# lxvm/AutoBZCore.jl

Hardware: AMD Instinct MI355X
Metric: k-point evals/sec (H(k)+eig) (higher is better)
Workload: dtype f64

## Files before the change

autobzcore.jl_amd/csrc/abz_internal.h:

```cpp
#pragma once
#include <hip/hip_ext.h>
#include <hip/hip_runtime.h>

#include <atomic>
#include <cstdint>
#include <cstdio>
#include <memory>
#include <string>
#include <vector>

#include "../../include/abzhip.h"
#include "dev_buf.h"
#include "ltm_block.h"
#include "plane_view.h"

namespace abz {
struct ProfScope;
struct RulePlan;

void set_error(const char* fmt, ...);
int catch_status() noexcept;

#define ABZ_CATCH_ALL \
    catch (...) { return abz::catch_status(); }
// ... 28 lines not shown
    SW_IPANEL_FMAC,
    SW_GGR_FUSED,
    SW_GGR_FUSE2,
    SW_GGR_UNIFORM,
    SW_IAI_SPECULATE,
    SW_IAI_PACKED,
    SW_IAI_POOL_MB,
    SW_IAI_DEVICE_INNER,
    SW_IAI_PANELS,
    SW_IAI_STATS,
    SW_HOST_THREADS,
    SW_AUTO_SWEEP_MAPPED,
    SW_LANE_KERNELS,
    SW_BIG_MFMA,
    SW_BIG_CHUNK_MB,
    SW_BIG_TRI_WAVES,
    SW_EIG_FOLD,
    SW_EIG_SPLIT,
    SW_IAI_LANES,
    SW_IAI_LANE_MIN,
    SW_CHAIN_FUSED,
    SW_EVAL_FUSED,
    SW_EVAL_PAIRS,
    SW_COUNT
};
int abz_switch(Switch s);

int stage_h2d(abz_ctx* ctx, void* dst_dev, const void* src_host, size_t bytes);
int stage_d2h(abz_ctx* ctx, void* dst_host, const void* src_dev, size_t bytes);
int mbox_reserve(abz_ctx* ctx);

int sweep_to_device(abz_ctx* ctx, const double* host, int n, const double** dev);

struct SumOut {
    double* host = nullptr;
    double* dev = nullptr;
    double2* map_dev = nullptr;
    const double2* map_host = nullptr;
};
int sum_target(abz_ctx* ctx, const SumOut& so, int64_t col0, int64_t ncols, double2** where);
int sum_deliver(abz_ctx* ctx, const SumOut& so, const double2* from, int64_t col0, int64_t ncols);

struct EnergyList {
    std::vector<int> perm;
    std::vector<double> Es, res;
    const double* dev = nullptr;
// ... 65 lines not shown
        so.map_dev = mbox_results<double2>(ctx, true);
        so.map_host = mbox_results<const double2>(ctx, false);
    }
    return so;
}
struct SeriesRule {
    int npt = 0, want = 0;
    std::vector<int32_t> syms;
    abz_rule* r = nullptr;
    uint64_t generation = 0;
    uint64_t stamp = 0;
};
}

struct abz_series {
    std::atomic<int> refs{1};
    bool closed = false;
    abz_ctx* ctx = nullptr;
    int d = 0, n = 0;
    int dims[ABZ_MAX_DIM] = {1, 1, 1};
    int first[ABZ_MAX_DIM] = {0, 0, 0};
    double period[ABZ_MAX_DIM] = {1, 1, 1};
    bool hermitian = false;
    int pivoting = ABZ_PIVOT_NONE;
    abz::DevBuf coef_pk;
    bool coef_pk_valid = false;
    abz::DevBuf coef;
    std::vector<abz_series*> lanes;
    abz::DevBuf pool[ABZ_MAX_DIM + 1];
    abz::DevBuf iai_pool[ABZ_MAX_DIM + 1];
    int64_t iai_used[ABZ_MAX_DIM + 1] = {0, 0, 0, 0};
    abz::DevBuf iai_io[6];
    abz_exchange_fn ex_fn = nullptr;
    void* ex_user = nullptr;
    int ex_rank = 0, ex_world = 1;
    void* iai_pin[5] = {nullptr, nullptr, nullptr, nullptr, nullptr};
    size_t iai_pin_cap[5] = {0, 0, 0, 0, 0};
    void* iai_pin_dev[5] = {nullptr, nullptr, nullptr, nullptr, nullptr};
    uint64_t generation = 0;
    std::vector<abz::SeriesRule> kept_rules;
    uint64_t kept_stamp = 0;
    std::vector<int> summed_once;
    uint64_t auto_hint_key = 0;
    int auto_hint_grids = 0;
    abz::DevBuf auto_io;
    void* auto_pin = nullptr;
// ... 104 lines not shown
                          int64_t L, int M3, int M2, int npt, int gbeg, int gcnt);

struct EvalSpec {
    int n;
    int M, first;
    double period;
    const double2* src;
    bool grid;
    int npt;
    int64_t nlines;
    const double2* tab;
    int64_t nk;
    const int64_t* run_start = nullptr;
    int64_t nruns = 0;
    const int64_t* parents;
    const int32_t* gi;
    const double* x;
    bool deriv;
    bool herm;
    bool packed = false;
    const double2* src2 = nullptr;
    const double2* phs2 = nullptr;
    int M2 = 0;
    PlaneView H;
    PlaneView E;
    PlaneView U;
};
int launch_eval(abz_ctx* ctx, const EvalSpec& es);
bool eval_packed_supported(int n, int M, int npt);
bool eval_fused_supported(int n, int64_t mnn, int M2, int npt, bool pairs = false);
int launch_pack_rows(abz_ctx* ctx, int n, int M, const double2* src, int64_t nrows, double2* out);
size_t packed_row_elems(int n, int M);
int series_ensure_packed(abz_series* s);

int launch_eig_planes(abz_ctx* ctx, int n, PlaneView H, PlaneView E, PlaneView U, int64_t nk);
int launch_velocity(abz_ctx* ctx, int n, PlaneView U, PlaneView dH, PlaneView Vj, int64_t nk);

struct ReduceSpec {
    int n, d, npt;
    int integrand;
    PlaneView H;
    PlaneView E;
    int64_t nk;
    const double* w;
    const int32_t* idx;
    int64_t k_offset = 0;
    bool herm = false;
    bool pivot = false;
    double params[4];
    const double* sweep_dev;
    int n_sweep;
    double scale;
// ... 238 lines not shown
```

autobzcore.jl_amd/csrc/api.cpp:

```cpp
#include <algorithm>
#include <atomic>
#include <cstdarg>
#include <chrono>
#include <cmath>
#include <cstring>
#include <map>
#include <mutex>
#include <numeric>
#include <thread>

#include "abz_internal.h"

namespace abz {

static thread_local std::string g_err;

void set_error(const char* fmt, ...) {
    char buf[1024];
    va_list ap;
    va_start(ap, fmt);
    vsnprintf(buf, sizeof(buf), fmt, ap);
    va_end(ap);
    g_err = buf;
}
// ... 40 lines not shown
    {"ABZ_IPANEL_FMAC", 1, "0: 16-lane panel kernel with separate pivot-row broadcasts"},
    {"ABZ_GGR_FUSED", 1, "0: GGR build by eigenvectors + one velocity launch per variable"},
    {"ABZ_GGR_FUSE2", 1, "0: fused GGR build reads level-1 families instead of contracting variable 2 itself"},
    {"ABZ_GGR_UNIFORM", 1, "0: GGR scans search the energy window even in equispaced lists"},
    {"ABZ_IAI_SPECULATE", 1, "0: nested IAI driver requests one panel per integral and round"},
    {"ABZ_IAI_PACKED", 1, "0: IAI chains on plain coefficient sets"},
    {"ABZ_IAI_POOL_MB", 0, "> 0: MB per chunk of level sets in the IAI driver (default: sized from free memory)"},
    {"ABZ_IAI_DEVICE_INNER", 1, "0: innermost GK loops driven from the host, one launch per round"},
    {"ABZ_IAI_PANELS", 1, "0: the level above the innermost one ships nodes instead of panels (GK rule of that level on the host)"},
    {"ABZ_IAI_STATS", 0, "1: per-solve statistics of the IAI driver on stderr"},
    {"ABZ_HOST_THREADS", 8, "host threads for the per-integral bookkeeping of IAI sweeps (capped at half the cores)"},
    {"ABZ_AUTO_SWEEP_MAPPED", 1, "0: abz_autoptr_solve* uploads its swept values instead of letting the kernels read the pinned host copy"},
    {"ABZ_LANE_KERNELS", 1, "0: 5...8-band rule builds / store-free sums on full grids through the 8-lane row kernels (test: same values)"},
    {"ABZ_BIG_MFMA", 0, "1: 33...64 bands: the level-1 evaluation of full grid lines as a real GEMM on v_mfma_f64_16x16x4_f64 (test: same values)"},
    {"ABZ_BIG_CHUNK_MB", 0, "33...64 bands: MB of scratch for the matrices of a chunk of nodes (0: 256, GGR builds 2048; tests set 1 to walk many chunks)"},
    {"ABZ_BIG_TRI_WAVES", 0, "33...64 bands: waves per node of the Householder tridiagonalisation (1, 2, 4: the same reflectors, another summation order; 0: two up to 44 bands, one up to 48, four above)"},
    {"ABZ_EIG_FOLD", 1, "0: 5...16-band rule builds evaluate the full level-1 series of a Hermitian model instead of the folded one"},
    {"ABZ_EIG_SPLIT", 1, "0: eigenvalues of 5...16-band rules by bisection inside the grid kernel instead of the per-lane QR kernel"},
    {"ABZ_IAI_LANES", 4, "lanes (host thread + stream each) a sweep of independent IAI solves is split over; 1: off"},
    {"ABZ_IAI_LANE_MIN", 16, "solves per lane below which a sweep is not split further"},
    {"ABZ_CHAIN_FUSED", 1, "0: 3-D full-grid chains contract variables 3 and 2 in two launches instead of contract_chain_kernel"},
    {"ABZ_EVAL_FUSED", 1, "0: 3-D full-grid rules (n <= 4) build level-1 sets with contract_chain_kernel instead of contracting variable 2 inside the grid kernel"},
    {"ABZ_EVAL_PAIRS", 1, "fused grid kernel, one grid line per half-wave: 1 where it takes fewer lane-rounds per line (Hermitian series), 0 never, 2 wherever supported (tests: same values)"},
};
}

int abz_switch(Switch s) {
    const char* e = getenv(g_switches[s].name);
    return (e && *e) ? atoi(e) : g_switches[s].dflt;
}

namespace {
struct Block {
    void* p;
    size_t cap;
    int device;
};
std::mutex g_pool_mutex;
std::vector<Block> g_pool;
size_t g_pool_bytes = 0;
std::atomic<int64_t> g_live_bytes{0};
std::atomic<int64_t> g_live_blocks{0};
size_t pool_limit() {
    static const size_t lim = (size_t)std::max(0, abz_switch(SW_POOL_MB)) << 20;
    return lim;
}
// ... 673 lines not shown
    return ABZ_OK;
} ABZ_CATCH_ALL

int abz_prof_reset(abz_ctx* ctx) try {
    ABZ_REQUIRE(ctx, "null ctx");
    int rc = prof_collect(ctx);
    for (auto& sl : ctx->prof_slots) {
        sl.ms = 0;
        sl.launches = 0;
    }
    return rc;
} ABZ_CATCH_ALL

int abz_prof_read(abz_ctx* ctx, int kernel_id, double* total_ms, int64_t* launches) try {
    ABZ_REQUIRE(ctx && kernel_id >= 0 && kernel_id < ABZ_K_COUNT, "bad profile slot");
    int rc = prof_collect(ctx);
    if (rc) return rc;
    if (total_ms) *total_ms = ctx->prof_slots[kernel_id].ms;
    if (launches) *launches = ctx->prof_slots[kernel_id].launches;
    return ABZ_OK;
} ABZ_CATCH_ALL

static bool detect_hermitian(const abz_series* s, const double* coef_reim);

int abz_series_create(abz_ctx* ctx, const double* coef_reim, int d, const int32_t* dims, const int32_t* first,
                      const double* period, int n, abz_series** out) try {
    ABZ_REQUIRE(ctx && coef_reim && dims && first && period && out, "abz_series_create: null argument");
    ABZ_REQUIRE(!ctx->closed, "abz_series_create: the context was destroyed");
    ABZ_REQUIRE(d >= 1 && d <= ABZ_MAX_DIM, "series dimension d = %d not in 1..%d", d, ABZ_MAX_DIM);
    ABZ_REQUIRE(n >= 1 && n <= ABZ_MAX_BANDS, "n = %d bands not in 1..%d", n, ABZ_MAX_BANDS);
    *out = nullptr;
    ABZ_HIP(hipSetDevice(ctx->device));
    std::unique_ptr<abz_series> s(new abz_series());
    s->ctx = ctx;
    s->d = d;
    s->n = n;
    for (int j = 0; j < d; ++j) {
        ABZ_REQUIRE(dims[j] >= 1 && period[j] > 0, "dims[%d] = %d / period = %g invalid", j, dims[j], period[j]);
        s->dims[j] = dims[j];
        s->first[j] = first[j];
        s->period[j] = period[j];
    }
    const size_t bytes = sizeof(double2) * (size_t)s->elems(d);
    if (s->coef.alloc(bytes)) return ABZ_ERR_NOMEM;
    hipError_t e = hipMemcpy(s->coef.p, coef_reim, bytes, hipMemcpyHostToDevice);
    if (e != hipSuccess) {
        set_error("coefficient upload failed: %s", hipGetErrorString(e));
        return ABZ_ERR_HIP;
    }
    s->hermitian = detect_hermitian(s.get(), coef_reim);
    ctx->refs += 1;
    *out = s.release();
    return ABZ_OK;
} ABZ_CATCH_ALL

static bool detect_hermitian(const abz_series* s, const double* coef_reim) {
    const int d = s->d, n = s->n;
    for (int j = 0; j < d; ++j)
        if (s->first[j] != -(s->dims[j] - 1) - s->first[j]) return false;
    int64_t nR = 1;
    for (int j = 0; j < d; ++j) nR *= s->dims[j];
    const int nn = n * n;
    for (int64_t r = 0; r < nR; ++r) {
        int64_t rem = r, mr = 0, mul = 1;
        for (int j = 0; j < d; ++j) {
            const int64_t i = rem % s->dims[j];
            rem /= s->dims[j];
            mr += (s->dims[j] - 1 - i) * mul;
            mul *= s->dims[j];
        }
        if (mr < r) continue;
        const double* A = coef_reim + 2 * r * nn;
        const double* B = coef_reim + 2 * mr * nn;
        for (int b = 0; b < n; ++b)
            for (int a = 0; a < n; ++a) {
                if (A[2 * (a + n * b)] != B[2 * (b + n * a)] || A[2 * (a + n * b) + 1] != -B[2 * (b + n * a) + 1])
                    return false;
            }
    }
    return true;
}

int abz_series_update(abz_series* s, const double* coef_reim) try {
    int rc = check_series(s);
    if (rc) return rc;
    ABZ_REQUIRE(coef_reim, "null coefficients");
    ABZ_HIP(hipSetDevice(s->ctx->device));
    ABZ_HIP(hipMemcpyAsync(s->coef.p, coef_reim, sizeof(double2) * (size_t)s->elems(s->d), hipMemcpyHostToDevice,
                           s->ctx->stream));
    ABZ_HIP(hipStreamSynchronize(s->ctx->stream));
    s->hermitian = detect_hermitian(s, coef_reim);
    s->coef_pk_valid = false;
    s->generation += 1;
    for (int64_t& u : s->iai_used) u = 0;
    for (abz_series* v : s->lanes) {
        v->hermitian = s->hermitian;
        v->coef_pk_valid = false;
        v->generation += 1;
    }
    return ABZ_OK;
} ABZ_CATCH_ALL

int abz_series_set_pivoting(abz_series* s, int mode) try {
    ABZ_REQUIRE(s, "abz_series_set_pivoting: null series");
    int rc = check_series(s);
    if (rc) return rc;
    ABZ_REQUIRE(mode == ABZ_PIVOT_NONE || mode == ABZ_PIVOT_PARTIAL, "abz_series_set_pivoting: mode %d is neither ABZ_PIVOT_NONE nor ABZ_PIVOT_PARTIAL", mode);
    s->pivoting = mode;
    for (abz_series* v : s->lanes) v->pivoting = mode;
    return ABZ_OK;
} ABZ_CATCH_ALL

int abz_series_get_pivoting(const abz_series* s, int* mode) try {
    ABZ_REQUIRE(s && mode, "abz_series_get_pivoting: null argument");
    ABZ_REQUIRE(!s->closed, "abz_series_get_pivoting: the series was destroyed");
    *mode = s->pivoting;
    return ABZ_OK;
} ABZ_CATCH_ALL

}

namespace abz {
int series_lane_views(abz_series* s, int count) {
    while ((int)s->lanes.size() < count) {
        abz_ctx* c = nullptr;
        int rc = abz_ctx_create(s->ctx->device, &c);
        if (rc) return rc;
        abz_series* v = new abz_series();
        v->ctx = c;
        v->d = s->d;
        v->n = s->n;
        for (int j = 0; j < ABZ_MAX_DIM; ++j) {
            v->dims[j] = s->dims[j];
            v->first[j] = s->first[j];
            v->period[j] = s->period[j];
        }
        v->hermitian = s->hermitian;
        v->pivoting = s->pivoting;
        v->coef = DevBuf::view_of(s->coef.p);
        c->refs += 1;
        s->lanes.push_back(v);
    }
    return ABZ_OK;
}
}

extern "C" {

static void series_drop_kept_rules(abz_series* s) {
    if (s->kept_rules.empty()) return;
    (void)hipSetDevice(s->ctx->device);
    (void)hipStreamSynchronize(s->ctx->stream);
    for (auto& k : s->kept_rules) delete k.r;
    s->kept_rules.clear();
    s->summed_once.clear();
}

int abz_series_destroy(abz_series* s) try {
    if (!s || s->closed) return ABZ_OK;
    series_drop_kept_rules(s);
// ... 173 lines not shown
        es.first = s->first[0];
        es.period = s->period[0];
        es.src = level1;
        if (level2) {
            es.src2 = level2;
            es.phs2 = rp->pd.phg[1].as<double2>();
            es.M2 = s->dims[1];
        }
        es.grid = r->full;
        es.npt = r->npt;
        es.nlines = r->full ? (d == 1 ? 1 : plan.nitems[1]) : 0;
        es.tab = tab;
        es.nk = r->nk;
        es.parents = r->full ? nullptr : rp->pd.parent[0].as<int64_t>();
        es.gi = r->full ? nullptr : rp->pd.gi[0].as<int32_t>();
        if (!r->full && plan.nruns > 0 && !plan.coords) {
            es.run_start = rp->pd.runs.as<int64_t>();
            es.nruns = plan.nruns;
        }
        es.x = nullptr;
        es.deriv = deriv;
        es.herm = s->hermitian;
        es.packed = packed_chain && !deriv && !Uout.base;
        es.H = Hout;
        es.E = Eout;
        es.U = Uout;
        return launch_eval(ctx, es);
    };
    const double2* level1 = nullptr;
    int rc;
    const int64_t line_elems = packed_chain ? (int64_t)packed_row_elems(n, s->dims[0]) : (int64_t)s->dims[0] * n * n;
    const bool ref_layout_large = s->hermitian && r->H.base && !r->H.compact && r->npt > 64;
    const bool eval_fused = r->full && d == 3 && n <= 4 && !(r->want & ABZ_WANT_VEL) && !Uv.base && rp->pd.phg[2].p && rp->pd.phg[1].p &&
                            !ref_layout_large &&
                            abz_switch(SW_CHAIN_FUSED) && abz_switch(SW_EVAL_FUSED) &&
                            contract_chain_fits(line_elems, s->dims[2], s->dims[1], r->npt, plan.outer_n) &&
                            eval_fused_supported(n, line_elems, s->dims[1], r->npt);
    if (eval_fused) {
        const double2* level2 = nullptr;
        if ((rc = build_chain(s, plan, rp->pd, tab, 0, &level2, 2, nullptr, packed_chain))) return rc;
        return run_eval(nullptr, false, r->H, r->E, PlaneView(), level2);
    }
    if ((rc = build_chain(s, plan, rp->pd, tab, 0, &level1, 1, nullptr, packed_chain))) return rc;
    if ((rc = run_eval(level1, false, r->H, vel_done ? PlaneView() : r->E, Uv))) return rc;
    if ((r->want & ABZ_WANT_VEL) && !vel_done) {
        for (int j = 1; j <= d; ++j) {
// ... 886 lines not shown
```

autobzcore.jl_amd/csrc/kernels.hip:

```cpp
#include "abz_internal.h"
#include "device_math.h"
#include "gk15.h"
#include "inner_adapt.h"
#include "packed_herm.h"

#include <cmath>
#include <cstring>
#include <type_traits>
#include <utility>
#include <cstdlib>

namespace abz {

static inline int64_t cdiv(int64_t a, int64_t b) { return (a + b - 1) / b; }

struct cplx_pod {
    double x, y;
};
typedef const cplx_pod __attribute__((address_space(4))) * cptr_t;
__device__ __forceinline__ cptr_t as_const(const double2* p) {
    return (cptr_t)(unsigned long long)p;
}

struct PhaseArgs {
// ... 442 lines not shown
        for (int a = 0; a < N; ++a) {
            H.re[a][b] = in[(int64_t)(2 * (a + N * b)) * v.pitch];
            H.im[a][b] = in[(int64_t)(2 * (a + N * b) + 1) * v.pitch];
        }
    }
}

struct EvalArgs {
    const double2* src;
    const double2* tab;
    const int64_t* parents;
    const int32_t* gi;
    const double* x;
    PlaneView H, E, U;
    int64_t nlines, nk;
    int64_t line0;
    int M, first, npt, deriv, herm;
    int nt;
    int pk;
    double inv_period;
    const double2* src2 = nullptr;
    const double2* phs2 = nullptr;
    int M2 = 0, bpk = 0;
};

template <bool NT>
__device__ __forceinline__ void store_f64(double* p, double v) {
    if constexpr (NT)
        __builtin_nontemporal_store(v, p);
    else
        *p = v;
}
template <int N, bool NT = false, bool HC = false>
__device__ __forceinline__ void store_planes_at(const CMat<N>& H, const PlaneView& v, int64_t line, int i1) {
    double* __restrict__ row = v.base + line * v.tile;
    const unsigned u = (unsigned)i1;
    if constexpr (HC) {
#pragma unroll
        for (int b = 0; b < N; ++b) {
#pragma unroll
            for (int a = 0; a <= b; ++a) {
                store_f64<NT>((row + (int64_t)(b * b + 2 * a) * v.pitch) + u, H.re[a][b]);
                if (a < b) store_f64<NT>((row + (int64_t)(b * b + 2 * a + 1) * v.pitch) + u, H.im[a][b]);
            }
        }
    } else {
#pragma unroll
        for (int b = 0; b < N; ++b) {
#pragma unroll
            for (int a = 0; a < N; ++a) {
                store_f64<NT>((row + (int64_t)(2 * (a + N * b)) * v.pitch) + u, H.re[a][b]);
                store_f64<NT>((row + (int64_t)(2 * (a + N * b) + 1) * v.pitch) + u, H.im[a][b]);
            }
        }
    }
}

template <int N, bool VEC = true>
__device__ __forceinline__ void eval_epilogue(const EvalArgs& a, CMat<N>& H, int64_t line, int i1) {
    if (a.H.base) {
        if (a.H.compact)
            store_planes_at<N, false, true>(H, a.H, line, i1);
        else
            store_planes_at<N>(H, a.H, line, i1);
    }
    if (a.E.base || (VEC && a.U.base)) {
        double e[N];
        CMat<N> V;
        if (VEC && a.U.base) {
            herm_eig<N, true>(H, e, V);
            store_planes_at<N>(V, a.U, line, i1);
        } else {
            herm_eig_values<N>(H, e);
        }
        if (a.E.base) {
// ... 134 lines not shown
                    }
                }
            }
        }
#pragma unroll
        for (int j = 0; j < KPL; ++j) phase_step(pr[j], pi[j], zr[j], zi[j]);
    }
    mid();
#pragma unroll
    for (int j = 0; j < KPL; ++j) {
        if constexpr (HERM) {
#pragma unroll
            for (int bb = 0; bb < N; ++bb) {
#pragma unroll
                for (int aa = bb + 1; aa < N; ++aa) {
                    H[j].re[aa][bb] = H[j].re[bb][aa];
                    H[j].im[aa][bb] = -H[j].im[bb][aa];
                }
            }
        }
    }
}

template <int N, int KPL, bool VEC, int LW = 64>
__device__ __forceinline__ void eval_unit_store(const EvalArgs& a, CMat<N> (&H)[KPL], int i0, int lane, int64_t line, int off_h = 0,
                                                int off_e = 0, bool on = true) {
    if constexpr (VEC) {
        static_assert(LW == 64, "the pair mapping stores values and eigenvalues only");
#pragma unroll
        for (int j = 0; j < KPL; ++j) {
            const int i1 = i0 + lane + 64 * j;
            const int pitch = a.H.base ? a.H.row : a.E.row;
            if (i1 < pitch) eval_epilogue<N, VEC>(a, H[j], line, i1);
        }
    }
    if constexpr (!VEC) {
        const int pitch = a.H.base ? a.H.row : a.E.row;
        auto epilogue = [&](auto nt, auto hc) {
            constexpr bool NT = decltype(nt)::value;
            constexpr bool HC = decltype(hc)::value;
            if (a.H.base) {
#pragma unroll
                for (int j = 0; j < KPL; ++j) {
                    const int i1 = i0 + lane + LW * j;
                    if (i1 < pitch && on) store_planes_at<N, NT, HC>(H[j], a.H, line, i1 + off_h);
                }
            }
            if (a.E.base) {
#pragma unroll
                for (int j = 0; j < KPL; ++j) {
                    const int i1 = i0 + lane + LW * j;
                    if (i1 < pitch && on) {
                        double e[N];
                        herm_eig_values<N>(H[j], e);
                        double* __restrict__ row = a.E.base + line * a.E.tile;
                        const unsigned u = (unsigned)(i1 + off_e);
#pragma unroll
                        for (int b = 0; b < N; ++b) store_f64<NT>((row + (int64_t)b * a.E.pitch) + u, e[b]);
                    }
                }
            }
        };
        if (a.H.compact) {
            if (a.nt)
                epilogue(std::true_type{}, std::true_type{});
            else
                epilogue(std::false_type{}, std::true_type{});
        } else if (a.nt)
            epilogue(std::true_type{}, std::false_type{});
        else
            epilogue(std::false_type{}, std::false_type{});
    }
}

template <int N, int KPL, bool HERM, bool VEC, class MID, bool PK = false, int LW = 64>
__device__ __forceinline__ void eval_unit(const EvalArgs& a, const double2* __restrict__ c1, const double2* tab_l, int fm,
                                          const int (&iz0)[KPL], const int (&iw0)[KPL], int npass, int i0, int lane,
                                          int64_t line, MID&& mid, int off_h = 0, int off_e = 0, bool on = true) {
    CMat<N> H[KPL];
    eval_unit_core<N, KPL, HERM, MID&, PK, LW>(a, c1, tab_l, fm, iz0, iw0, npass, i0, lane, mid, H);
    eval_unit_store<N, KPL, VEC, LW>(a, H, i0, lane, line, off_h, off_e, on);
}

__device__ __forceinline__ void wave_lds_sync() {
    __builtin_amdgcn_fence(__ATOMIC_RELEASE, "wavefront");
    __builtin_amdgcn_wave_barrier();
    __builtin_amdgcn_fence(__ATOMIC_ACQUIRE, "wavefront");
}

struct LinePhases {
    double x[ABZ_CONTRACT_GRID_MAXM], y[ABZ_CONTRACT_GRID_MAXM];
};
__device__ __forceinline__ void load_line_phases(cptr_t p, LinePhases& ph) {
#pragma unroll
    for (int m = 0; m < ABZ_CONTRACT_GRID_MAXM; ++m) {
        ph.x[m] = p[m].x;
        ph.y[m] = p[m].y;
    }
}

template <int M2>
__device__ __forceinline__ void contract_line(const double2* s2, const LinePhases& ph, double2* dst, int MNN, int lane) {
    for (int l = lane; l < MNN; l += 64) {
        double ar = 0.0, ai = 0.0;
#pragma unroll
        for (int m = 0; m < M2; ++m) {
            const double2 c = s2[m * MNN + l];
            ar = fma(c.x, ph.x[m], ar);
            ar = fma(-c.y, ph.y[m], ar);
            ai = fma(c.x, ph.y[m], ai);
            ai = fma(c.y, ph.x[m], ai);
        }
        dst[l] = make_double2(ar, ai);
    }
}

__device__ __forceinline__ void contract_line_m(int M2, const double2* s2, const LinePhases& ph, double2* dst, int MNN, int lane) {
#define CL(MM) case MM: contract_line<MM>(s2, ph, dst, MNN, lane); break;
    switch (M2) {
        CL(1) CL(2) CL(3) CL(4) CL(5) CL(6) CL(7) CL(8) CL(9) CL(10) CL(11) CL(12) CL(13) CL(14) CL(15) CL(16)
        default: break;
    }
#undef CL
}

template <int N, int KPL, bool HERM, bool VEC, int OCC, bool PK = false, bool FUSE = false, bool PAIR = false, int KT = KPL>
__global__ __launch_bounds__(256, OCC) void eval_grid_kernel(EvalArgs a) {
    static_assert(FUSE || !PAIR, "the pair mapping exists in the fused instance only");
    static_assert(KT >= 1 && KT <= KPL && (PAIR || KT == KPL), "a shorter last pass exists in the pair mapping only");
    constexpr int LPU = PAIR ? 2 : 1;
    extern __shared__ double2 lds_c[];
    const int wave = __builtin_amdgcn_readfirstlane(threadIdx.x >> 6), lane = threadIdx.x & 63;
    const int MNN = PK ? Pk<N>::size((a.M - 1) / 2) : a.M * N * N;
    auto stage = [&](double2 c, int idx) -> double2 {
        if (!a.deriv) return c;
        const double f = 6.283185307179586476925286766559 * (double)(a.first + idx / (N * N));
        return make_double2(-f * c.y, f * c.x);
    };
    double2* const mybuf = lds_c + (size_t)wave * 2 * LPU * MNN;
    int fm = a.first % a.npt;
    if (fm < 0) fm += a.npt;
    constexpr int LW = 64 / LPU;
    const int npass = (a.npt + LW * KPL - 1) / (LW * KPL);
    double2* const tab_l = lds_c + (size_t)4 * 2 * LPU * MNN;
    if constexpr (FUSE) {
        static_assert(!VEC, "the fused instance stores values and eigenvalues only");
        const int k3 = blockIdx.y, seg = blockIdx.x;
        const int L2 = a.M2 * MNN;
        const double2* __restrict__ src2 = a.src2 + (int64_t)k3 * L2;
        double2* const s2 = tab_l + a.npt;
        const int kstride = 4 * a.bpk;
        int k2 = LPU * (4 * seg + wave);
        LinePhases ph;
        load_line_phases(as_const(a.phs2 + (int64_t)(k2 < a.npt ? k2 : 0) * a.M2), ph);
        {
            const int it = threadIdx.x;
            double2 vt = a.tab[min(it, a.npt - 1)];
            double2 v[4];
#pragma unroll
            for (int j = 0; j < 4; ++j) v[j] = src2[min(it + 256 * j, L2 - 1)];
            asm volatile("" : "+v"(vt.x), "+v"(vt.y));
#pragma unroll
            for (int j = 0; j < 4; ++j) asm volatile("" : "+v"(v[j].x), "+v"(v[j].y));
            if (it < a.npt) tab_l[it] = vt;
#pragma unroll
            for (int j = 0; j < 4; ++j)
                if (it + 256 * j < L2) s2[it + 256 * j] = v[j];
            for (int i = it + 256; i < a.npt; i += 256) tab_l[i] = a.tab[i];
            for (int i = it + 4 * 256; i < L2; i += 256) s2[i] = src2[i];
        }
// ... 16 lines not shown
                }
            }
            const int off_h = half * (int)a.H.tile, off_e = half * (int)a.E.tile;
            int cur = 0, pass = 0;
            while (k2 < a.npt) {
                const bool last_pass = pass + 1 >= npass;
                const int nk2 = last_pass ? k2 + 2 * kstride : k2;
                const bool contract_next = last_pass && nk2 < a.npt;
                wave_lds_sync();
                auto mid_fn = [&]() __attribute__((always_inline)) {
                    if (contract_next) {
                        int ln = lane;
                        asm volatile("" : "+v"(ln));
                        double2* const dst = mybuf + (size_t)(cur ^ 1) * 2 * MNN;
                        load_line_phases(as_const(a.phs2 + (int64_t)nk2 * a.M2), ph);
                        contract_line_m(a.M2, s2, ph, dst, MNN, ln);
                        load_line_phases(as_const(a.phs2 + (int64_t)min(nk2 + 1, a.npt - 1) * a.M2), ph);
                        contract_line_m(a.M2, s2, ph, dst + MNN, MNN, ln);
                    }
                };
                const double2* const c1 = mybuf + (size_t)(2 * cur + half) * MNN;
                const int64_t line = (int64_t)k3 * a.npt + k2;
                const bool on = half == 0 || k2 + 1 < a.npt;
                if constexpr (KT == KPL) {
                    eval_unit<N, KPL, HERM, VEC, decltype(mid_fn)&, PK, 32>(a, c1, tab_l, fm, iz0, iw0, npass, pass * (32 * KPL), col, line, mid_fn,
                                                                            off_h, off_e, on);
                } else if (!last_pass) {
                    auto no_mid = []() {};
                    eval_unit<N, KPL, HERM, VEC, decltype(no_mid)&, PK, 32>(a, c1, tab_l, fm, iz0, iw0, npass, pass * (32 * KPL), col, line, no_mid,
                                                                            off_h, off_e, on);
                } else {
                    eval_unit<N, KT, HERM, VEC, decltype(mid_fn)&, PK, 32>(a, c1, tab_l, fm, izt, iwt, npass, pass * (32 * KPL), col, line, mid_fn,
                                                                           off_h, off_e, on);
                }
                if (last_pass) cur ^= 1;
                pass = last_pass ? 0 : pass + 1;
                k2 = nk2;
            }
            return;
        }
        int iz0[KPL], iw0[KPL];
#pragma unroll
        for (int j = 0; j < KPL; ++j) {
            const int i1 = lane + 64 * j;
            iz0[j] = i1 < a.npt ? i1 : 0;
            iw0[j] = (int)(((unsigned)fm * (unsigned)iz0[j]) % (unsigned)a.npt);
        }
        int cur = 0, pass = 0;
        while (k2 < a.npt) {
            const bool last_pass = pass + 1 >= npass;
            const int nk2 = last_pass ? k2 + kstride : k2;
            const bool contract_next = last_pass && nk2 < a.npt;
            wave_lds_sync();
            auto mid_fn = [&]() {
                if (contract_next) {
                    load_line_phases(as_const(a.phs2 + (int64_t)nk2 * a.M2), ph);
                    contract_line_m(a.M2, s2, ph, mybuf + (size_t)(cur ^ 1) * MNN, MNN, lane);
                }
            };
            eval_unit<N, KPL, HERM, VEC, decltype(mid_fn)&, PK>(a, mybuf + (size_t)cur * MNN, tab_l, fm, iz0, iw0, npass, pass * (64 * KPL), lane,
                                                                (int64_t)k3 * a.npt + k2, mid_fn);
            if (last_pass) cur ^= 1;
            pass = last_pass ? 0 : pass + 1;
            k2 = nk2;
        }
        return;
    }
    for (int i = threadIdx.x; i < a.npt; i += 256) tab_l[i] = a.tab[i];
    __syncthreads();
    const int64_t lstride = (int64_t)gridDim.x * 4;
    int64_t line = (int64_t)blockIdx.x * 4 + wave;
    if (line >= a.nlines) return;
    {
        const double2* __restrict__ src = a.src + line * MNN;
#pragma unroll
        for (int t = 0; t < EVAL_MAX_MNN / 64; ++t) {
            const int idx = lane + 64 * t;
            if (idx < MNN) mybuf[idx] = stage(src[idx], idx);
        }
    }
    int iz0[KPL], iw0[KPL];
#pragma unroll
    for (int j = 0; j < KPL; ++j) {
        const int i1 = lane + 64 * j;
// ... 7 lines not shown
        const bool have_next = nline < a.nlines;
        double2 pre[EVAL_MAX_MNN / 64];
        {
            const double2* __restrict__ src = a.src + (have_next ? nline : line) * MNN;
#pragma unroll
            for (int t = 0; t < EVAL_MAX_MNN / 64; ++t) {
                const int idx = lane + 64 * t;
                pre[t] = src[idx < MNN ? idx : MNN - 1];
            }
        }
        wave_lds_sync();
        auto mid_fn = [&]() {
#pragma unroll
            for (int t = 0; t < EVAL_MAX_MNN / 64; ++t) asm volatile("" : "+v"(pre[t].x), "+v"(pre[t].y));
            if (have_next) {
                double2* dst = mybuf + (size_t)(cur ^ 1) * MNN;
#pragma unroll
                for (int t = 0; t < EVAL_MAX_MNN / 64; ++t) {
                    const int idx = lane + 64 * t;
                    if (idx < MNN) dst[idx] = stage(pre[t], idx);
                }
            }
        };
        eval_unit<N, KPL, HERM, VEC, decltype(mid_fn)&, PK>(a, mybuf + (size_t)cur * MNN, tab_l, fm, iz0, iw0, npass, pass * (64 * KPL), lane, line,
                                                            mid_fn);
        cur ^= 1;
        pass = last_pass ? 0 : pass + 1;
        line = nline;
    }
}

template <int N>
__global__ __launch_bounds__(256) void eval_grid_kernel_scalar(EvalArgs a) {
    const int wave = threadIdx.x >> 6, lane = threadIdx.x & 63;
    int fm = a.first % a.npt;
    if (fm < 0) fm += a.npt;
    for (int64_t line = (int64_t)blockIdx.x * 4 + wave; line < a.nlines; line += (int64_t)gridDim.x * 4) {
        const unsigned lo = __builtin_amdgcn_readfirstlane((unsigned)(line & 0xffffffffu));
        const unsigned hi = __builtin_amdgcn_readfirstlane((unsigned)((unsigned long long)line >> 32));
        const int64_t line_u = (int64_t)(((unsigned long long)hi << 32) | lo);
        cptr_t c1 = as_const(a.src + line_u * ((int64_t)a.M * N * N));
        for (int i0 = 0; i0 < a.npt; i0 += 64) {
            const int i1 = i0 + lane;
            if (i1 < a.npt) {
                const double2 z = a.tab[i1];
                const double2 w = a.tab[(int)(((int64_t)fm * i1) % a.npt)];
                CMat<N> H;
                series_lane<N>(c1, a.M, a.first, z.x, z.y, w.x, w.y, a.deriv != 0, H);
// ... 33 lines not shown
}

#define ABZ_DISPATCH_N(n, FN)                                       \
    switch (n) {                                                    \
        case 1: FN(1); break;                                       \
        case 2: FN(2); break;                                       \
        case 3: FN(3); break;                                       \
        case 4: FN(4); break;                                       \
        default:                                                    \
            set_error("n = %d bands: only n <= 4 is built in this round", n); \
            return ABZ_ERR_UNSUPPORTED;                             \
    }

bool eval_packed_supported(int n, int M, int npt) {
    if (!abz_switch(SW_EVAL_PACKED) || n < 1 || n > 4 || (M & 1) == 0) return false;
    const size_t P = packed_row_elems(n, M);
    return P <= (size_t)EVAL_MAX_MNN && npt < 65536 && sizeof(double2) * (4 * 2 * P + (size_t)npt) <= 64 * 1024;
}

bool eval_fused_supported(int n, int64_t mnn, int M2, int npt, bool pairs) {
    const size_t lpu = pairs ? 2 : 1;
    return n >= 1 && n <= 4 && mnn >= 1 && mnn <= EVAL_MAX_MNN && M2 >= 1 && M2 <= ABZ_CONTRACT_GRID_MAXM && npt >= 1 &&
           npt < 65536 && sizeof(double2) * ((size_t)M2 * mnn + 4 * 2 * lpu * (size_t)mnn + (size_t)npt) <= 64 * 1024;
}

int launch_eval(abz_ctx* ctx, const EvalSpec& es) {
    if (es.n > 4) {
        GenSpec gs;
        gs.Uplanes = es.U;
        gs.herm = es.herm && !es.deriv;
        gs.n = es.n;
        gs.M = es.M;
        gs.first = es.first;
        gs.npt = es.npt;
        gs.d = 0;
        gs.period = es.period;
        gs.src = es.src;
        gs.grid = es.grid;
        gs.parents = es.parents;
        gs.run_start = es.run_start;
        gs.nruns = es.nruns;
        gs.gi = es.gi;
        gs.x = es.x;
        gs.tab = es.tab;
        gs.deriv = es.deriv;
        gs.nnodes = es.grid ? es.nlines * es.npt : es.nk;
// ... 39 lines not shown
        if (es.nlines == 0) return ABZ_OK;
        const int64_t quads = cdiv(es.nlines, 4);
        const int64_t blocks = std::min<int64_t>(quads, quads < 5000 ? 256 * 8 : (es.H.compact ? 256 * 24 : 256 * 16));
        const int mnn = a.pk ? es.n * (es.n + 1) / 2 + ((es.M - 1) / 2) * es.n * es.n : es.M * es.n * es.n;
        int kpl = 1;
        {
            double best = 1e30;
            for (int k = 1; k <= 3; ++k) {
                const double cost = (double)(cdiv(es.npt, 64 * k) * k) * (1.0 + 0.3 / k);
                if (cost < best - 1e-12) {
                    best = cost;
                    kpl = k;
                }
            }
        }
        const size_t lds = sizeof(double2) * (4 * 2 * (size_t)mnn + (size_t)a.npt);
        if (es.src2) {
            if (es.deriv || es.U.base || !eval_fused_supported(es.n, mnn, es.M2, es.npt) || es.nlines % es.npt != 0 ||
                es.nlines / es.npt > 65535) {
                set_error("eval: fused contraction unsupported (n = %d, %d numbers per line, M2 = %d, npt = %d)", es.n, mnn, es.M2, es.npt);
                return ABZ_ERR_UNSUPPORTED;
            }
            const int64_t gcnt = es.nlines / es.npt;
            a.src2 = es.src2;
            a.phs2 = es.phs2;
            a.M2 = es.M2;
            if (ctx->prof & (1u << ABZ_K_EVAL_FUSED)) ctx->prof_slots[ABZ_K_EVAL_FUSED].launches += 1;
            a.bpk = (int)std::max<int64_t>(1, std::min<int64_t>(cdiv(es.npt, 4), cdiv(blocks, gcnt)));
            a.bpk = (int)cdiv(es.npt, 4 * cdiv(es.npt, 4 * a.bpk));
            const size_t flds = lds + sizeof(double2) * (size_t)es.M2 * mnn;
            const int sw_pairs = abz_switch(SW_EVAL_PAIRS);
            const int rounds = (int)cdiv(es.npt, 32);
            const bool pairs = sw_pairs != 0 && eval_fused_supported(es.n, mnn, es.M2, es.npt, true) && es.H.tile < INT32_MAX &&
                               es.E.tile < INT32_MAX && (sw_pairs >= 2 || (a.herm && rounds < 2 * cdiv(es.npt, 64 * kpl) * kpl));
            if (pairs) {
                const int kp = es.n < 4 ? 3 : (a.herm ? 2 : 1);
                const int kt = rounds - (int)(cdiv(rounds, kp) - 1) * kp;
                const int64_t npairs = cdiv(es.npt, 2);
                a.bpk = (int)std::max<int64_t>(1, std::min<int64_t>(cdiv(npairs, 4), cdiv(blocks, gcnt)));
                a.bpk = (int)cdiv(npairs, 4 * cdiv(npairs, 4 * a.bpk));
                const size_t plds = flds + sizeof(double2) * 4 * 2 * (size_t)mnn;
                const dim3 grid((unsigned)a.bpk, (unsigned)gcnt);
#define LKP(NN, KT)                                                                                                          \
    {                                                                                                                        \
        constexpr int OO = NN == 3 ? 3 : 2;                                                                                  \
        constexpr int KH = NN < 4 ? 3 : 2, KG = NN < 4 ? 3 : 1;                                                \
        if (a.pk)                                                                                                            \
            launch(ctx, eval_grid_kernel<NN, KH, true, false, OO, true, true, true, KT <= KH ? KT : KH>, grid, dim3(256), plds, a);  \
        else if (a.herm)                                                                                                     \
            launch(ctx, eval_grid_kernel<NN, KH, true, false, OO, false, true, true, KT <= KH ? KT : KH>, grid, dim3(256), plds, a); \
        else                                                                                                                 \
            launch(ctx, eval_grid_kernel<NN, KG, false, false, 2, false, true, true, KT <= KG ? KT : KG>, grid, dim3(256), plds, a); \
    }
#define FN(NN)                     \
    switch (kt) {                  \
        case 1: LKP(NN, 1) break;  \
        case 2: LKP(NN, 2) break;  \
        default: LKP(NN, 3) break; \
    }
                ABZ_DISPATCH_N(es.n, FN)
#undef FN
#undef LKP
            } else {
#define LK(NN, KK)                                                                                                                         \
    {                                                                                                                                      \
        constexpr int OO = NN == 3 ? 3 : 2;                                                                                                \
        if (a.pk)                                                                                                                          \
            launch(ctx, eval_grid_kernel<NN, KK, true, false, OO, true, true>, dim3((unsigned)a.bpk, (unsigned)gcnt), dim3(256), flds, a);  \
        else if (a.herm)                                                                                                                   \
            launch(ctx, eval_grid_kernel<NN, KK, true, false, OO, false, true>, dim3((unsigned)a.bpk, (unsigned)gcnt), dim3(256), flds, a); \
        else                                                                                                                               \
            launch(ctx, eval_grid_kernel<NN, KK, false, false, 2, false, true>, dim3((unsigned)a.bpk, (unsigned)gcnt), dim3(256), flds, a); \
    }
#define FN(NN)                    \
    switch (kpl) {                \
        case 1: LK(NN, 1) break;  \
        case 2: LK(NN, 2) break;  \
        default: LK(NN, 3) break; \
    }
            ABZ_DISPATCH_N(es.n, FN)
#undef FN
#undef LK
            }
        } else if (mnn <= EVAL_MAX_MNN && lds <= 64 * 1024 && a.npt < 65536) {
#define LK(NN, KK)                                                                                                             \
    {                                                                                                                          \
        constexpr int OO = NN == 3 ? 3 : 2;                                                                                    \
        if (a.pk)                                                                                                              \
            launch(ctx, eval_grid_kernel<NN, KK, true, false, OO, true>, dim3((unsigned)blocks), dim3(256), lds, a); \
        else if (a.U.base)                                                                                                     \
            launch(ctx, eval_grid_kernel<NN, KK, false, true, 2>, dim3((unsigned)blocks), dim3(256), lds, a);  \
        else if (a.herm)                                                                                                       \
            launch(ctx, eval_grid_kernel<NN, KK, true, false, OO>, dim3((unsigned)blocks), dim3(256), lds, a); \
        else                                                                                                                   \
            launch(ctx, eval_grid_kernel<NN, KK, false, false, 2>, dim3((unsigned)blocks), dim3(256), lds, a); \
    }
#define FN(NN)                    \
    switch (kpl) {                \
        case 1: LK(NN, 1) break;  \
        case 2: LK(NN, 2) break;  \
        default: LK(NN, 3) break; \
    }
            ABZ_DISPATCH_N(es.n, FN)
#undef FN
#undef LK
        } else {
#define FN(NN) launch(ctx, eval_grid_kernel_scalar<NN>, dim3((unsigned)blocks), dim3(256), 0, a)
            ABZ_DISPATCH_N(es.n, FN)
#undef FN
        }
    } else {
        if (es.nk == 0) return ABZ_OK;
        const int64_t blocks = cdiv(es.nk, 256);
#define FN(NN) launch(ctx, eval_node_kernel<NN>, dim3((unsigned)blocks), dim3(256), 0, a)
        ABZ_DISPATCH_N(es.n, FN)
#undef FN
    }
    ABZ_HIP(hipGetLastError());
// ... 1811 lines not shown
```

Before: 47.34 billion.

## Mirror H(-k)=conj H(k) for real Hermitian series on full 3-D grids

Detects series whose coefficients are all real. When such a series is also Hermitian, the 3-D full-grid evaluation kernels compute only the planes with k3 <= npt/2 and write the conjugated matrices and the same eigenvalues to the mirrored k-point. This roughly halves the series evaluation and eigen work, while the number of output stores stays the same and the extra mirrored writes are scattered. A size threshold, adjustable by a switch, limits the mirror path to launches that write at most 600 MB.

```diff
diff --git a/autobzcore.jl_amd/csrc/abz_internal.h b/autobzcore.jl_amd/csrc/abz_internal.h
--- a/autobzcore.jl_amd/csrc/abz_internal.h
+++ b/autobzcore.jl_amd/csrc/abz_internal.h
@@ -74,6 +74,7 @@
     SW_CHAIN_FUSED,
     SW_EVAL_FUSED,
     SW_EVAL_PAIRS,
+    SW_EVAL_MIRROR,
     SW_COUNT
 };
 int abz_switch(Switch s);
@@ -185,6 +186,7 @@
     int first[ABZ_MAX_DIM] = {0, 0, 0};
     double period[ABZ_MAX_DIM] = {1, 1, 1};
     bool hermitian = false;
+    bool real_coef = false;
     int pivoting = ABZ_PIVOT_NONE;
     abz::DevBuf coef_pk;
     bool coef_pk_valid = false;
@@ -335,12 +337,14 @@
     const double2* src2 = nullptr;
     const double2* phs2 = nullptr;
     int M2 = 0;
+    bool mirror = false;
     PlaneView H;
     PlaneView E;
     PlaneView U;
 };
 int launch_eval(abz_ctx* ctx, const EvalSpec& es);
 bool eval_packed_supported(int n, int M, int npt);
+bool eval_mirror_supported(const EvalSpec& es);
 bool eval_fused_supported(int n, int64_t mnn, int M2, int npt, bool pairs = false);
 int launch_pack_rows(abz_ctx* ctx, int n, int M, const double2* src, int64_t nrows, double2* out);
 size_t packed_row_elems(int n, int M);
diff --git a/autobzcore.jl_amd/csrc/api.cpp b/autobzcore.jl_amd/csrc/api.cpp
--- a/autobzcore.jl_amd/csrc/api.cpp
+++ b/autobzcore.jl_amd/csrc/api.cpp
@@ -86,6 +86,7 @@
     {"ABZ_CHAIN_FUSED", 1, "0: 3-D full-grid chains contract variables 3 and 2 in two launches instead of contract_chain_kernel"},
     {"ABZ_EVAL_FUSED", 1, "0: 3-D full-grid rules (n <= 4) build level-1 sets with contract_chain_kernel instead of contracting variable 2 inside the grid kernel"},
     {"ABZ_EVAL_PAIRS", 1, "fused grid kernel, one grid line per half-wave: 1 where it takes fewer lane-rounds per line (Hermitian series), 0 never, 2 wherever supported (tests: same values)"},
+    {"ABZ_EVAL_MIRROR", 1, "3-D full-grid rules (n <= 4) of a real Hermitian series evaluate the planes k3 <= npt/2 and store H(-k) = conj H(k) beside them: 1 where the launch writes at most 600 MB, 0 never (every plane evaluated), 2 wherever supported"},
 };
 }
 
@@ -805,6 +806,7 @@
 } ABZ_CATCH_ALL
 
 static bool detect_hermitian(const abz_series* s, const double* coef_reim);
+static bool detect_real(const abz_series* s, const double* coef_reim);
 
 int abz_series_create(abz_ctx* ctx, const double* coef_reim, int d, const int32_t* dims, const int32_t* first,
                       const double* period, int n, abz_series** out) try {
@@ -832,6 +834,7 @@
         return ABZ_ERR_HIP;
     }
     s->hermitian = detect_hermitian(s.get(), coef_reim);
+    s->real_coef = detect_real(s.get(), coef_reim);
     ctx->refs += 1;
     *out = s.release();
     return ABZ_OK;
@@ -864,6 +867,13 @@
     return true;
 }
 
+static bool detect_real(const abz_series* s, const double* coef_reim) {
+    const int64_t cnt = s->elems(s->d);
+    for (int64_t i = 0; i < cnt; ++i)
+        if (coef_reim[2 * i + 1] != 0.0) return false;
+    return true;
+}
+
 int abz_series_update(abz_series* s, const double* coef_reim) try {
     int rc = check_series(s);
     if (rc) return rc;
@@ -873,11 +883,13 @@
                            s->ctx->stream));
     ABZ_HIP(hipStreamSynchronize(s->ctx->stream));
     s->hermitian = detect_hermitian(s, coef_reim);
+    s->real_coef = detect_real(s, coef_reim);
     s->coef_pk_valid = false;
     s->generation += 1;
     for (int64_t& u : s->iai_used) u = 0;
     for (abz_series* v : s->lanes) {
         v->hermitian = s->hermitian;
+        v->real_coef = s->real_coef;
         v->coef_pk_valid = false;
         v->generation += 1;
     }
@@ -919,6 +931,7 @@
             v->period[j] = s->period[j];
         }
         v->hermitian = s->hermitian;
+        v->real_coef = s->real_coef;
         v->pivoting = s->pivoting;
         v->coef = DevBuf::view_of(s->coef.p);
         c->refs += 1;
@@ -1138,6 +1151,12 @@
         es.deriv = deriv;
         es.herm = s->hermitian;
         es.packed = packed_chain && !deriv && !Uout.base;
+        const int sw_mirror = abz_switch(SW_EVAL_MIRROR);
+        const PlaneView& pv = Hout.base ? Hout : Eout;
+        const double out_bytes = 8.0 * ((Hout.base ? (Hout.compact ? 1.0 : 2.0) * n * n : 0.0) + (Eout.base ? (double)n : 0.0)) *
+                                 (double)pv.row * (double)es.nlines;
+        es.mirror = s->hermitian && s->real_coef && r->full && d == 3 && plan.outer_n == r->npt && !deriv && !Uout.base &&
+                    !(r->want & ABZ_WANT_VEL) && (sw_mirror >= 2 || (sw_mirror == 1 && out_bytes <= 600e6));
         es.H = Hout;
         es.E = Eout;
         es.U = Uout;
diff --git a/autobzcore.jl_amd/csrc/kernels.hip b/autobzcore.jl_amd/csrc/kernels.hip
--- a/autobzcore.jl_amd/csrc/kernels.hip
+++ b/autobzcore.jl_amd/csrc/kernels.hip
@@ -488,6 +488,7 @@
     const double2* src2 = nullptr;
     const double2* phs2 = nullptr;
     int M2 = 0, bpk = 0;
+    int mirror = 0;
 };
 
 template <bool NT>
@@ -497,7 +498,7 @@
     else
         *p = v;
 }
-template <int N, bool NT = false, bool HC = false>
+template <int N, bool NT = false, bool HC = false, bool CONJ = false>
 __device__ __forceinline__ void store_planes_at(const CMat<N>& H, const PlaneView& v, int64_t line, int i1) {
     double* __restrict__ row = v.base + line * v.tile;
     const unsigned u = (unsigned)i1;
@@ -507,7 +508,7 @@
 #pragma unroll
             for (int a = 0; a <= b; ++a) {
                 store_f64<NT>((row + (int64_t)(b * b + 2 * a) * v.pitch) + u, H.re[a][b]);
-                if (a < b) store_f64<NT>((row + (int64_t)(b * b + 2 * a + 1) * v.pitch) + u, H.im[a][b]);
+                if (a < b) store_f64<NT>((row + (int64_t)(b * b + 2 * a + 1) * v.pitch) + u, CONJ ? -H.im[a][b] : H.im[a][b]);
             }
         }
     } else {
@@ -516,7 +517,7 @@
 #pragma unroll
             for (int a = 0; a < N; ++a) {
                 store_f64<NT>((row + (int64_t)(2 * (a + N * b)) * v.pitch) + u, H.re[a][b]);
-                store_f64<NT>((row + (int64_t)(2 * (a + N * b) + 1) * v.pitch) + u, H.im[a][b]);
+                store_f64<NT>((row + (int64_t)(2 * (a + N * b) + 1) * v.pitch) + u, (CONJ && a != b) ? -H.im[a][b] : H.im[a][b]);
             }
         }
     }
@@ -697,9 +698,14 @@
     }
 }
 
+struct MirrorTo {
+    int64_t line = -1;
+    int t0 = 0, t1 = 0;
+};
+
 template <int N, int KPL, bool VEC, int LW = 64>
 __device__ __forceinline__ void eval_unit_store(const EvalArgs& a, CMat<N> (&H)[KPL], int i0, int lane, int64_t line, int off_h = 0,
-                                                int off_e = 0, bool on = true) {
+                                                int off_e = 0, bool on = true, const MirrorTo mt = MirrorTo()) {
     if constexpr (VEC) {
         static_assert(LW == 64, "the pair mapping stores values and eigenvalues only");
 #pragma unroll
@@ -711,6 +717,14 @@
     }
     if constexpr (!VEC) {
         const int pitch = a.H.base ? a.H.row : a.E.row;
+        const bool mir = mt.line >= 0;
+        auto moffset = [&](int j, int64_t tile) {
+            int tx = threadIdx.x;
+            asm volatile("" : "+v"(tx));
+            const int i1 = i0 + (tx & (LW - 1)) + LW * j;
+            const int mc = (i1 == 0 || i1 >= a.npt) ? i1 : a.npt - i1;
+            return mc + (LW == 32 && (tx & 32) ? mt.t1 : mt.t0) * (int)tile;
+        };
         auto epilogue = [&](auto nt, auto hc) {
             constexpr bool NT = decltype(nt)::value;
             constexpr bool HC = decltype(hc)::value;
@@ -719,6 +733,13 @@
                 for (int j = 0; j < KPL; ++j) {
                     const int i1 = i0 + lane + LW * j;
                     if (i1 < pitch && on) store_planes_at<N, NT, HC>(H[j], a.H, line, i1 + off_h);
+                }
+                if (mir) {
+#pragma unroll
+                    for (int j = 0; j < KPL; ++j) {
+                        const int i1 = i0 + lane + LW * j;
+                        if (i1 < pitch && on) store_planes_at<N, false, HC, true>(H[j], a.H, mt.line, moffset(j, a.H.tile));
+                    }
                 }
             }
             if (a.E.base) {
@@ -732,6 +753,12 @@
                         const unsigned u = (unsigned)(i1 + off_e);
 #pragma unroll
                         for (int b = 0; b < N; ++b) store_f64<NT>((row + (int64_t)b * a.E.pitch) + u, e[b]);
+                        if (mir) {
+                            double* __restrict__ mrow = a.E.base + mt.line * a.E.tile;
+                            const unsigned mu = (unsigned)moffset(j, a.E.tile);
+#pragma unroll
+                            for (int b = 0; b < N; ++b) store_f64<false>((mrow + (int64_t)b * a.E.pitch) + mu, e[b]);
+                        }
                     }
                 }
             }
@@ -751,10 +778,11 @@
 template <int N, int KPL, bool HERM, bool VEC, class MID, bool PK = false, int LW = 64>
 __device__ __forceinline__ void eval_unit(const EvalArgs& a, const double2* __restrict__ c1, const double2* tab_l, int fm,
                                           const int (&iz0)[KPL], const int (&iw0)[KPL], int npass, int i0, int lane,
-                                          int64_t line, MID&& mid, int off_h = 0, int off_e = 0, bool on = true) {
+                                          int64_t line, MID&& mid, int off_h = 0, int off_e = 0, bool on = true,
+                                          const MirrorTo mt = MirrorTo()) {
     CMat<N> H[KPL];
     eval_unit_core<N, KPL, HERM, MID&, PK, LW>(a, c1, tab_l, fm, iz0, iw0, npass, i0, lane, mid, H);
-    eval_unit_store<N, KPL, VEC, LW>(a, H, i0, lane, line, off_h, off_e, on);
+    eval_unit_store<N, KPL, VEC, LW>(a, H, i0, lane, line, off_h, off_e, on, mt);
 }
 
 __device__ __forceinline__ void wave_lds_sync() {
@@ -799,8 +827,9 @@
 #undef CL
 }
 
-template <int N, int KPL, bool HERM, bool VEC, int OCC, bool PK = false, bool FUSE = false, bool PAIR = false, int KT = KPL>
+template <int N, int KPL, bool HERM, bool VEC, int OCC, bool PK = false, bool FUSE = false, bool PAIR = false, int KT = KPL, bool MIR = false>
 __global__ __launch_bounds__(256, OCC) void eval_grid_kernel(EvalArgs a) {
+    static_assert(!MIR || (HERM && !VEC), "mirrored launches: values and eigenvalues of a Hermitian series");
     static_assert(FUSE || !PAIR, "the pair mapping exists in the fused instance only");
     static_assert(KT >= 1 && KT <= KPL && (PAIR || KT == KPL), "a shorter last pass exists in the pair mapping only");
     constexpr int LPU = PAIR ? 2 : 1;
@@ -821,6 +850,7 @@
     if constexpr (FUSE) {
         static_assert(!VEC, "the fused instance stores values and eigenvalues only");
         const int k3 = blockIdx.y, seg = blockIdx.x;
+        const int mk3 = (MIR && k3 != 0 && 2 * k3 != a.npt) ? a.npt - k3 : -1;
         const int L2 = a.M2 * MNN;
         const double2* __restrict__ src2 = a.src2 + (int64_t)k3 * L2;
         double2* const s2 = tab_l + a.npt;
@@ -883,16 +913,22 @@
                 const double2* const c1 = mybuf + (size_t)(2 * cur + half) * MNN;
                 const int64_t line = (int64_t)k3 * a.npt + k2;
                 const bool on = half == 0 || k2 + 1 < a.npt;
+                MirrorTo mt;
+                if (mk3 >= 0) {
+                    mt.line = (int64_t)mk3 * a.npt;
+                    mt.t0 = k2 ? a.npt - k2 : 0;
+                    mt.t1 = k2 + 1 < a.npt ? a.npt - k2 - 1 : 0;
+                }
                 if constexpr (KT == KPL) {
                     eval_unit<N, KPL, HERM, VEC, decltype(mid_fn)&, PK, 32>(a, c1, tab_l, fm, iz0, iw0, npass, pass * (32 * KPL), col, line, mid_fn,
-                                                                            off_h, off_e, on);
+                                                                            off_h, off_e, on, mt);
                 } else if (!last_pass) {
                     auto no_mid = []() {};
                     eval_unit<N, KPL, HERM, VEC, decltype(no_mid)&, PK, 32>(a, c1, tab_l, fm, iz0, iw0, npass, pass * (32 * KPL), col, line, no_mid,
-                                                                            off_h, off_e, on);
+                                                                            off_h, off_e, on, mt);
                 } else {
                     eval_unit<N, KT, HERM, VEC, decltype(mid_fn)&, PK, 32>(a, c1, tab_l, fm, izt, iwt, npass, pass * (32 * KPL), col, line, mid_fn,
-                                                                           off_h, off_e, on);
+                                                                           off_h, off_e, on, mt);
                 }
                 if (last_pass) cur ^= 1;
                 pass = last_pass ? 0 : pass + 1;
@@ -919,8 +955,10 @@
                     contract_line_m(a.M2, s2, ph, mybuf + (size_t)(cur ^ 1) * MNN, MNN, lane);
                 }
             };
+            MirrorTo mt;
+            if (mk3 >= 0) mt.line = (int64_t)mk3 * a.npt + (k2 ? a.npt - k2 : 0);
             eval_unit<N, KPL, HERM, VEC, decltype(mid_fn)&, PK>(a, mybuf + (size_t)cur * MNN, tab_l, fm, iz0, iw0, npass, pass * (64 * KPL), lane,
-                                                                (int64_t)k3 * a.npt + k2, mid_fn);
+                                                                (int64_t)k3 * a.npt + k2, mid_fn, 0, 0, true, mt);
             if (last_pass) cur ^= 1;
             pass = last_pass ? 0 : pass + 1;
             k2 = nk2;
@@ -974,8 +1012,13 @@
                 }
             }
         };
+        MirrorTo mt;
+        if constexpr (MIR) {
+            const unsigned k3 = (unsigned)line / (unsigned)a.npt, k2 = (unsigned)line - k3 * (unsigned)a.npt;
+            if (k3 != 0 && 2 * (int)k3 != a.npt) mt.line = (int64_t)(a.npt - (int)k3) * a.npt + (k2 ? a.npt - (int)k2 : 0);
+        }
         eval_unit<N, KPL, HERM, VEC, decltype(mid_fn)&, PK>(a, mybuf + (size_t)cur * MNN, tab_l, fm, iz0, iw0, npass, pass * (64 * KPL), lane, line,
-                                                            mid_fn);
+                                                            mid_fn, 0, 0, true, mt);
         cur ^= 1;
         pass = last_pass ? 0 : pass + 1;
         line = nline;
@@ -1055,6 +1098,23 @@
     const size_t lpu = pairs ? 2 : 1;
     return n >= 1 && n <= 4 && mnn >= 1 && mnn <= EVAL_MAX_MNN && M2 >= 1 && M2 <= ABZ_CONTRACT_GRID_MAXM && npt >= 1 &&
            npt < 65536 && sizeof(double2) * ((size_t)M2 * mnn + 4 * 2 * lpu * (size_t)mnn + (size_t)npt) <= 64 * 1024;
+}
+
+template <class F>
+static void with_flags(bool p, bool q, F&& f) {
+    if (p)
+        q ? f(std::true_type{}, std::true_type{}) : f(std::true_type{}, std::false_type{});
+    else
+        q ? f(std::false_type{}, std::true_type{}) : f(std::false_type{}, std::false_type{});
+}
+
+bool eval_mirror_supported(const EvalSpec& es) {
+    if (!es.mirror || !es.grid || !es.herm || es.deriv || es.U.base || es.n < 1 || es.n > 4 || es.npt < 1 || es.npt >= 65536 ||
+        es.nlines != (int64_t)es.npt * es.npt || es.nlines >= INT32_MAX)
+        return false;
+    for (const PlaneView* v : {&es.H, &es.E})
+        if (v->base && ((int64_t)es.npt * v->tile + v->row >= INT32_MAX || v->tile < 0)) return false;
+    return true;
 }
 
 int launch_eval(abz_ctx* ctx, const EvalSpec& es) {
@@ -1140,6 +1200,8 @@
                 return ABZ_ERR_UNSUPPORTED;
             }
             const int64_t gcnt = es.nlines / es.npt;
+            a.mirror = eval_mirror_supported(es) ? 1 : 0;
+            const unsigned grows = a.mirror ? (unsigned)(es.npt / 2 + 1) : (unsigned)gcnt;
             a.src2 = es.src2;
             a.phs2 = es.phs2;
             a.M2 = es.M2;
@@ -1158,15 +1220,15 @@
                 a.bpk = (int)std::max<int64_t>(1, std::min<int64_t>(cdiv(npairs, 4), cdiv(blocks, gcnt)));
                 a.bpk = (int)cdiv(npairs, 4 * cdiv(npairs, 4 * a.bpk));
                 const size_t plds = flds + sizeof(double2) * 4 * 2 * (size_t)mnn;
-                const dim3 grid((unsigned)a.bpk, (unsigned)gcnt);
+                const dim3 grid((unsigned)a.bpk, grows);
 #define LKP(NN, KT)                                                                                                          \
     {                                                                                                                        \
         constexpr int OO = NN == 3 ? 3 : 2;                                                                                  \
         constexpr int KH = NN < 4 ? 3 : 2, KG = NN < 4 ? 3 : 1;                                                \
-        if (a.pk)                                                                                                            \
-            launch(ctx, eval_grid_kernel<NN, KH, true, false, OO, true, true, true, KT <= KH ? KT : KH>, grid, dim3(256), plds, a);  \
-        else if (a.herm)                                                                                                     \
-            launch(ctx, eval_grid_kernel<NN, KH, true, false, OO, false, true, true, KT <= KH ? KT : KH>, grid, dim3(256), plds, a); \
+        if (a.herm)                                                                                                          \
+            with_flags(a.pk != 0, a.mirror != 0, [&](auto pk, auto mir) {                                                    \
+                launch(ctx, eval_grid_kernel<NN, KH, true, false, OO, pk(), true, true, KT <= KH ? KT : KH, mir()>, grid, dim3(256), plds, a); \
+            });                                                                                                              \
         else                                                                                                                 \
             launch(ctx, eval_grid_kernel<NN, KG, false, false, 2, false, true, true, KT <= KG ? KT : KG>, grid, dim3(256), plds, a); \
     }
@@ -1183,12 +1245,12 @@
 #define LK(NN, KK)                                                                                                                         \
     {                                                                                                                                      \
         constexpr int OO = NN == 3 ? 3 : 2;                                                                                                \
-        if (a.pk)                                                                                                                          \
-            launch(ctx, eval_grid_kernel<NN, KK, true, false, OO, true, true>, dim3((unsigned)a.bpk, (unsigned)gcnt), dim3(256), flds, a);  \
-        else if (a.herm)                                                                                                                   \
-            launch(ctx, eval_grid_kernel<NN, KK, true, false, OO, false, true>, dim3((unsigned)a.bpk, (unsigned)gcnt), dim3(256), flds, a); \
+        if (a.herm)                                                                                                                        \
+            with_flags(a.pk != 0, a.mirror != 0, [&](auto pk, auto mir) {                                                                  \
+                launch(ctx, eval_grid_kernel<NN, KK, true, false, OO, pk(), true, false, KK, mir()>, dim3((unsigned)a.bpk, grows), dim3(256), flds, a); \
+            });                                                                                                                            \
         else                                                                                                                               \
-            launch(ctx, eval_grid_kernel<NN, KK, false, false, 2, false, true>, dim3((unsigned)a.bpk, (unsigned)gcnt), dim3(256), flds, a); \
+            launch(ctx, eval_grid_kernel<NN, KK, false, false, 2, false, true>, dim3((unsigned)a.bpk, grows), dim3(256), flds, a); \
     }
 #define FN(NN)                    \
     switch (kpl) {                \
@@ -1201,17 +1263,22 @@
 #undef LK
             }
         } else if (mnn <= EVAL_MAX_MNN && lds <= 64 * 1024 && a.npt < 65536) {
+            if (eval_mirror_supported(es)) {
+                a.mirror = 1;
+                a.nlines = (int64_t)(es.npt / 2 + 1) * es.npt;
+            }
+            const unsigned lblocks = (unsigned)std::min<int64_t>(blocks, cdiv(a.nlines, 4));
 #define LK(NN, KK)                                                                                                             \
     {                                                                                                                          \
         constexpr int OO = NN == 3 ? 3 : 2;                                                                                    \
-        if (a.pk)                                                                                                              \
-            launch(ctx, eval_grid_kernel<NN, KK, true, false, OO, true>, dim3((unsigned)blocks), dim3(256), lds, a); \
-        else if (a.U.base)                                                                                                     \
-            launch(ctx, eval_grid_kernel<NN, KK, false, true, 2>, dim3((unsigned)blocks), dim3(256), lds, a);  \
+        if (a.U.base && !a.pk)                                                                                                 \
+            launch(ctx, eval_grid_kernel<NN, KK, false, true, 2>, dim3(lblocks), dim3(256), lds, a);                           \
         else if (a.herm)                                                                                                       \
-            launch(ctx, eval_grid_kernel<NN, KK, true, false, OO>, dim3((unsigned)blocks), dim3(256), lds, a); \
+            with_flags(a.pk != 0, a.mirror != 0, [&](auto pk, auto mir) {                                                      \
+                launch(ctx, eval_grid_kernel<NN, KK, true, false, OO, pk(), false, false, KK, mir()>, dim3(lblocks), dim3(256), lds, a); \
+            });                                                                                                                \
         else                                                                                                                   \
-            launch(ctx, eval_grid_kernel<NN, KK, false, false, 2>, dim3((unsigned)blocks), dim3(256), lds, a); \
+            launch(ctx, eval_grid_kernel<NN, KK, false, false, 2>, dim3(lblocks), dim3(256), lds, a);                          \
     }
 #define FN(NN)                    \
     switch (kpl) {                \
```

New measurement: 50.67 billion (median of 6 runs). +7.0%, better.
